# JOP-Lee/READ

Hardware: NVIDIA B200
Metric: frames/sec @1920x1080, 10M pts (higher is better)
Workload: dtype bf16

## Files before the change

read_b200/csrc/conv_tc.cu:

```cuda
#include "common.cuh"
#include "conv_common.cuh"
#include "ptx.cuh"
#include <cuda.h>
#include <mutex>
#include <new>

namespace rb {

#ifdef READ_DIAG
#define TC_DBG(a_, bit_) (((a_).debug & (bit_)) != 0)
#define TC_TRACE(role_, code_)                                                                                          \
    do {                                                                                                                \
        if (a.trace != nullptr && blockIdx.x == 0 && lane == 0 && trc_n < 2046u) {                                      \
            a.trace[(role_) * 2048 + 1 + trc_n] = ((unsigned long long)(code_) << 56) | ((unsigned long long)clock64() & 0x00FFFFFFFFFFFFFFull); \
            a.trace[(role_) * 2048] = ++trc_n;                                                                          \
        }                                                                                                               \
    } while (0)
#else
#define TC_DBG(a_, bit_) false
#define TC_TRACE(role_, code_) do { } while (0)
#endif

constexpr int TC_TW = 8, TC_TH = 16;
constexpr int TC_MAX_STAGES = 16;
constexpr uint32_t TC_SMEM_BUDGET = 218 * 1024;
constexpr uint32_t TC_RESIDENT_MAX = 144 * 1024;
constexpr int TC_TMEM_COLS = 512;
constexpr int TC_MAX_ACC = 8;
constexpr int BAR_AFULL = 0, BAR_AEMPTY = 16, BAR_BFULL = 32, BAR_BEMPTY = 48, BAR_TFULL = 64, BAR_TEMPTY = 72,
              BAR_BRES = 80, BAR_TMEMPTR = 82, BAR_RFULL = 84, BAR_PARAMS = 132;
constexpr int TC_STAGE_BYTES = 1024, TC_NBUF = 3;
constexpr uint32_t TC_STAGING_BYTES = 16u * TC_NBUF * TC_STAGE_BYTES;

struct TcMaps {
    CUtensorMap a[READ_MAX_SRC];
    CUtensorMap o, r;
};

struct TcArgs {
    int B, H, W, Cin, Cout, cout_pad;
    int ksize, pad;
    int cin_blk, kchunks;
    int n_tile, n_tiles;
    int tiles_x, tiles_y;
    int a_stages, b_stages, b_resident;
    int halo_w;
    uint32_t a_tx_bytes;
    uint32_t tile_bytes;
    int stride;
    int n_src;
    int src_kc_end[READ_MAX_SRC];
    int src_shift[READ_MAX_SRC];
    float inv_tx, inv_ty;
    int nacc;
    int dual;
    int debug;
    uint32_t a_bytes, b_bytes, b_region_off;
    int elu;
    const float *bias_f, *bias_m, *scale, *shift;
    const __nv_bfloat16 *residual;
    __nv_bfloat16 *out;
    float *out_nchw;
    __nv_bfloat16 *out2;
    const __nv_bfloat16 *out2_mul;
    const __nv_bfloat16 *addin;
    int addin_H, addin_W;
    int raw;
    int mt;
    int mt_log2, nacc_log2;
    int stiles_x;
    float inv_stx;
    int role_rot;
    int pdl;
    int commit_late;
    int merge_done;
    int bpair;
    int rev_total;
    int tma_out;
    uint32_t stage_bytes;
    int probe;
    unsigned long long *trace;
};

struct TileCoord {
    int nt, tx, ty, b;
};
__device__ __forceinline__ TileCoord decode_tile(long long t, const TcArgs &a)
{
    TileCoord c;
    if (a.rev_total) t = (long long)a.rev_total - 1 - t;
    int mt = (int)t;
    c.nt = 0;
    if (a.n_tiles == 2) { c.nt = mt & 1; mt >>= 1; }
    else if (a.n_tiles > 2) { c.nt = (int)(t % a.n_tiles); mt = (int)(t / a.n_tiles); }
    const int q = fdiv_small(mt, a.inv_stx);
    c.tx = (mt - q * a.stiles_x) * a.mt;
    c.b = fdiv_small(q, a.inv_ty);
    c.ty = q - c.b * a.tiles_y;
    return c;
}
__device__ __forceinline__ TileCoord decode_supertile(int s, const TcArgs &a)
{
    TileCoord c;
    c.nt = 0;
    if (a.rev_total) s = a.rev_total - 1 - s;
    const int q = fdiv_small(s, a.inv_stx);
    c.tx = (s - q * a.stiles_x) * a.mt;
    c.b = fdiv_small(q, a.inv_ty);
    c.ty = q - c.b * a.tiles_y;
    return c;
}
// ... 22 lines not shown
    extern __shared__ uint8_t smem_raw[];
    const uint32_t smem_base = (s_u32(smem_raw) + 1023u) & ~1023u;
    uint8_t *smem_al = smem_raw + (smem_base - s_u32(smem_raw));

    constexpr int ntaps = KS * KS;
    const uint32_t b_region = smem_base + a.b_region_off;
    const uint32_t b_region_bytes = RES ? (uint32_t)(ntaps * a.kchunks) * a.b_bytes : (uint32_t)a.b_stages * a.b_bytes;
    const uint32_t stage_region = smem_base + a.b_region_off + b_region_bytes;
    uint64_t *bars = reinterpret_cast<uint64_t *>(smem_al + a.b_region_off + b_region_bytes + a.stage_bytes);
    const uint32_t bar0 = s_u32(bars);
    const uint32_t afull0 = bar0 + 8 * BAR_AFULL, aempty0 = bar0 + 8 * BAR_AEMPTY;
    const uint32_t bfull0 = bar0 + 8 * BAR_BFULL, bempty0 = bar0 + 8 * BAR_BEMPTY;
    const uint32_t tfull0 = bar0 + 8 * BAR_TFULL, tempty0 = bar0 + 8 * BAR_TEMPTY, bres = bar0 + 8 * BAR_BRES;
    uint32_t *tmem_ptr_smem = reinterpret_cast<uint32_t *>(bars + BAR_TMEMPTR);
    float *s_par = reinterpret_cast<float *>(bars + BAR_PARAMS);

    const int lane = threadIdx.x & 31;
    const int warp = a.role_rot ? (int)(((threadIdx.x >> 5) + 4u) % (NTHR / 32)) : (int)(threadIdx.x >> 5);
    if (a.pdl) pdl_launch_dependents();
#ifdef READ_DIAG
    unsigned trc_n = 0;
#endif

    for (int i = threadIdx.x; i < a.cout_pad; i += NTHR) {
        const float hs = NTHR == 640 ? 0.5f : 1.f;
        reinterpret_cast<float4 *>(s_par)[i] = i < a.Cout ? make_float4(a.bias_f[i], hs * a.bias_m[i], hs * a.scale[i], a.shift[i])
                                                          : make_float4(0.f, 0.f, 0.f, 0.f);
    }
    if (warp == 0 && lane == 0) {
        for (int i = 0; i < a.n_src; ++i) tma_prefetch_desc(&tm.a[i]);
        tma_prefetch_desc(&tmB);
        if (a.tma_out) {
            tma_prefetch_desc(&tm.o);
            if (a.residual != nullptr) tma_prefetch_desc(&tm.r);
        }
    }
    if (warp == 1 && lane == 0) {
        for (int s = 0; s < TC_MAX_STAGES; ++s) {
            mbar_init(afull0 + 8 * s, 1);
            mbar_init(aempty0 + 8 * s, 1);
            mbar_init(bfull0 + 8 * s, 1);
            mbar_init(bempty0 + 8 * s, 1);
        }
        for (int i = 0; i < TC_MAX_ACC; ++i) {
            mbar_init(tfull0 + 8 * i, 1);
            mbar_init(tempty0 + 8 * i, NTHR == 640 ? (a.raw ? 16u : (uint32_t)(a.n_tile >> 3)) : ((a.n_tile >> 1) == 8 ? 4u : (NTHR - 128) / 32));
        }
        mbar_init(bres, 1);
        if (NTHR == 640)
            for (int i = 0; i < 16 * TC_NBUF; ++i) mbar_init(bar0 + 8 * (BAR_RFULL + i), 1);
        mbar_fence_init();
    }
    if (warp == 2) tmem_alloc(s_u32(tmem_ptr_smem), TC_TMEM_COLS);
    tcgen05_fence_before();
    __syncthreads();
    tcgen05_fence_after();
    const uint32_t tmem_base = *tmem_ptr_smem;

    const int m_tiles = a.stiles_x * a.tiles_y * a.B;
    const long long total_tiles = (long long)m_tiles * a.n_tiles;
    const int n_total = a.n_tile * a.n_tiles;

    if (warp == 0 || (warp == 2 && a.dual)) {
        const uint32_t pme = (warp == 2) ? 1u : 0u;
        if (RES && pme == 0u && elect_one()) {
            const int nb = KS * KS * a.kchunks;
            mbar_arrive_expect_tx(bres, (uint32_t)nb * a.b_bytes);
// ... 182 lines not shown
                        if (last_kc)
                            for (uint32_t mi = 0; mi < MT; ++mi) umma_commit(tfull0 + 8 * (acc + mi));
                    }
                    __syncwarp();
                }
                TC_TRACE(2 + me, 5);
                a_lo += st16;
                if (++as == ring_n) { as = 0; aph ^= 1u; a_lo = ring_lo0; }
            }
        }
    } else if (warp >= 4) {
        const int q = warp & 3;
        const int sub = (warp - 4) >> 2;
        const int r = q * 32 + lane;
        const int py = r / TC_TW, px = r % TC_TW;
        const int half = a.n_tile >> 1;
        const int nchunks = half >> 4;
        const float4 *par4 = reinterpret_cast<const float4 *>(s_par);
        unsigned tile_seq = 0;
        uint32_t acc_c = 0, acc_p = 0;
        if (a.pdl) pdl_wait();
        if (NTHR == 640 && (EPI != 0 || !a.raw)) {
            const bool elu = EPI == 1 ? true : (EPI == 2 ? false : a.elu != 0);
            const bool has_res = EPI == 2 ? true : (EPI == 1 ? false : a.residual != nullptr);
            const bool has_out2 = EPI != 0 ? false : a.out2 != nullptr;
            const int nch16 = half >> 4;
            const int lg = nch16 >> 1;
            const int chunk = sub & (nch16 - 1);
            const uint32_t item_step = 4u >> lg;
            const uint32_t n_units = (uint32_t)((total_tiles - blockIdx.x + gridDim.x - 1) / gridDim.x);
            const uint32_t n_mtiles = n_units << a.mt_log2;
            uint32_t acc = ((uint32_t)sub >> lg) % (uint32_t)a.nacc, acc_ph = (((uint32_t)sub >> lg) / (uint32_t)a.nacc) & 1u;
            const bool tma_out = a.tma_out != 0;
            const uint32_t sbuf0 = stage_region + (uint32_t)(warp - 4) * (TC_NBUF * TC_STAGE_BYTES);
            const uint32_t rfull0 = bar0 + 8 * (BAR_RFULL + (warp - 4) * TC_NBUF);
            const uint32_t lane_off = (uint32_t)lane * 32u, sw = (((uint32_t)lane >> 2) & 1u) * 16u;
            uint32_t kb = 0, kph = 0;
            if (tma_out && has_res && lane == 0 && ((uint32_t)sub >> lg) < n_mtiles) {
                const uint32_t it0 = (uint32_t)sub >> lg;
                const TileCoord t0 = decode_supertile((int)(blockIdx.x + (it0 >> a.mt_log2) * gridDim.x), a);
                mbar_arrive_expect_tx(rfull0, TC_STAGE_BYTES);
                tma_load_4d(&tm.r, rfull0, sbuf0, chunk * 16, (t0.tx + (int)(it0 & (uint32_t)(a.mt - 1))) * TC_TW, t0.ty * TC_TH + q * 4, t0.b);
            }
            for (uint32_t it = (uint32_t)sub >> lg; it < n_mtiles; it += item_step) {
                const uint32_t su = it >> a.mt_log2, mi = it & (uint32_t)(a.mt - 1);
                const TileCoord tc_ = decode_supertile((int)(blockIdx.x + su * gridDim.x), a);
                const int b = tc_.b;
                const int x = (tc_.tx + (int)mi) * TC_TW + px, y = tc_.ty * TC_TH + py;
                const bool inside = (x < a.W) && (y < a.H);
                const uint32_t trow = tmem_base + acc * (uint32_t)a.n_tile + ((uint32_t)(q * 32) << 16);
                const int co = chunk * 16;
                const int o = ((b * a.H + y) * a.W + x) * a.Cout + co;
                uint4 rs0 = make_uint4(0, 0, 0, 0), rs1 = rs0, ml0 = rs0, ml1 = rs0;
                uint4 af0 = rs0, af1 = rs0, am0 = rs0, am1 = rs0;
                const bool has_addin = EPI == 0 && a.addin != nullptr;
                if (has_addin && inside) {
                    const __nv_bfloat16 *ap = a.addin + ((b * a.addin_H + (y >> 1)) * a.addin_W + (x >> 1)) * a.n_tile + chunk * 16;
                    af0 = __ldg(reinterpret_cast<const uint4 *>(ap));
                    af1 = __ldg(reinterpret_cast<const uint4 *>(ap) + 1);
                    am0 = __ldg(reinterpret_cast<const uint4 *>(ap + half));
                    am1 = __ldg(reinterpret_cast<const uint4 *>(ap + half) + 1);
                }
                const uint32_t kn = kb + 1 == TC_NBUF ? 0u : kb + 1;
                if (tma_out) {
                    if (lane == 0) {
                        bulk_wait_group_read<1>();
                        const uint32_t itn = it + item_step;
                        if (has_res && itn < n_mtiles) {
                            const TileCoord tn = decode_supertile((int)(blockIdx.x + (itn >> a.mt_log2) * gridDim.x), a);
                            mbar_arrive_expect_tx(rfull0 + 8 * kn, TC_STAGE_BYTES);
                            tma_load_4d(&tm.r, rfull0 + 8 * kn, sbuf0 + kn * TC_STAGE_BYTES, co,
                                        (tn.tx + (int)(itn & (uint32_t)(a.mt - 1))) * TC_TW, tn.ty * TC_TH + q * 4, tn.b);
                        }
                    }
                } else if (inside) {
                    if (has_res) {
                        rs0 = __ldg(reinterpret_cast<const uint4 *>(a.residual + o));
                        rs1 = __ldg(reinterpret_cast<const uint4 *>(a.residual + o) + 1);
                    }
                    if (has_out2) {
                        ml0 = __ldg(reinterpret_cast<const uint4 *>(a.out2_mul + o));
                        ml1 = __ldg(reinterpret_cast<const uint4 *>(a.out2_mul + o) + 1);
                    }
                }
                TC_TRACE(warp, 9);
                mbar_wait(tfull0 + 8 * acc, acc_ph);
                TC_TRACE(warp, 6);
                tcgen05_fence_after();
                uint32_t f16[16], m16[16];
                tmem_ld16(trow + (uint32_t)(chunk * 16), f16);
                tmem_ld16(trow + (uint32_t)(half + chunk * 16), m16);
                tmem_ld_wait();
                TC_TRACE(warp, 7);
                tcgen05_fence_before();
                __syncwarp();
                if (lane == 0) mbar_arrive(tempty0 + 8 * acc);
                if (has_addin) {
                    const uint32_t fa[8] = {af0.x, af0.y, af0.z, af0.w, af1.x, af1.y, af1.z, af1.w};
                    const uint32_t ma[8] = {am0.x, am0.y, am0.z, am0.w, am1.x, am1.y, am1.z, am1.w};
#pragma unroll
                    for (int j = 0; j < 8; ++j) {
                        f16[2 * j] = __float_as_uint(__uint_as_float(f16[2 * j]) + __uint_as_float(fa[j] << 16));
                        f16[2 * j + 1] = __float_as_uint(__uint_as_float(f16[2 * j + 1]) + __uint_as_float(fa[j] & 0xFFFF0000u));
                        m16[2 * j] = __float_as_uint(__uint_as_float(m16[2 * j]) + __uint_as_float(ma[j] << 16));
                        m16[2 * j + 1] = __float_as_uint(__uint_as_float(m16[2 * j + 1]) + __uint_as_float(ma[j] & 0xFFFF0000u));
                    }
                }
                float yv[16];
                if (elu) {
#pragma unroll
                    for (int j = 0; j < 16; ++j) yv[j] = gate_folded<true>(__uint_as_float(f16[j]), __uint_as_float(m16[j]), par4[co + j]);
                } else {
#pragma unroll
                    for (int j = 0; j < 16; ++j) yv[j] = gate_folded<false>(__uint_as_float(f16[j]), __uint_as_float(m16[j]), par4[co + j]);
                }
                if (tma_out) {
                    const uint32_t sb = sbuf0 + kb * TC_STAGE_BYTES + lane_off;
                    if (has_res) {
                        mbar_wait(rfull0 + 8 * kb, kph);
                        asm volatile("ld.shared.v4.b32 {%0, %1, %2, %3}, [%4];" : "=r"(rs0.x), "=r"(rs0.y), "=r"(rs0.z), "=r"(rs0.w) : "r"(sb + sw));
                        asm volatile("ld.shared.v4.b32 {%0, %1, %2, %3}, [%4];" : "=r"(rs1.x), "=r"(rs1.y), "=r"(rs1.z), "=r"(rs1.w) : "r"(sb + (sw ^ 16u)));
                        const uint32_t rr[8] = {rs0.x, rs0.y, rs0.z, rs0.w, rs1.x, rs1.y, rs1.z, rs1.w};
#pragma unroll
                        for (int j = 0; j < 8; ++j) {
                            yv[2 * j] += __uint_as_float(rr[j] << 16);
                            yv[2 * j + 1] += __uint_as_float(rr[j] & 0xFFFF0000u);
                        }
                    }
                    uint32_t pk[8];
#pragma unroll
                    for (int j = 0; j < 8; ++j) pk[j] = cvt_bf16x2(yv[2 * j], yv[2 * j + 1]);
                    asm volatile("st.shared.v4.b32 [%0], {%1, %2, %3, %4};" ::"r"(sb + sw), "r"(pk[0]), "r"(pk[1]), "r"(pk[2]), "r"(pk[3]) : "memory");
                    asm volatile("st.shared.v4.b32 [%0], {%1, %2, %3, %4};" ::"r"(sb + (sw ^ 16u)), "r"(pk[4]), "r"(pk[5]), "r"(pk[6]), "r"(pk[7]) : "memory");
                    fence_proxy_async_smem();
                    __syncwarp();
                    if (lane == 0) {
                        if (!TC_DBG(a, 8)) tma_store_4d(&tm.o, sbuf0 + kb * TC_STAGE_BYTES, co, (tc_.tx + (int)mi) * TC_TW, tc_.ty * TC_TH + q * 4, b);
                        bulk_commit_group();
                    }
                    kb = kn;
                    if (kb == 0) kph ^= 1u;
                } else if (inside) {
                    if (has_res) {
                        const uint32_t rr[8] = {rs0.x, rs0.y, rs0.z, rs0.w, rs1.x, rs1.y, rs1.z, rs1.w};
#pragma unroll
                        for (int j = 0; j < 8; ++j) {
                            yv[2 * j] += __uint_as_float(rr[j] << 16);
                            yv[2 * j + 1] += __uint_as_float(rr[j] & 0xFFFF0000u);
                        }
                    }
                    uint32_t pk[8];
#pragma unroll
                    for (int j = 0; j < 8; ++j) pk[j] = cvt_bf16x2(yv[2 * j], yv[2 * j + 1]);
                    uint4 *op = reinterpret_cast<uint4 *>(a.out + o);
                    op[0] = make_uint4(pk[0], pk[1], pk[2], pk[3]);
                    op[1] = make_uint4(pk[4], pk[5], pk[6], pk[7]);
                    if (has_out2) {
                        const uint32_t mm[8] = {ml0.x, ml0.y, ml0.z, ml0.w, ml1.x, ml1.y, ml1.z, ml1.w};
                        uint32_t p2[8];
#pragma unroll
                        for (int j = 0; j < 8; ++j) {
                            const float2 ys = unpack_bf16x2(pk[j]);
                            const float2 mv = unpack_bf16x2(mm[j]);
                            p2[j] = cvt_bf16x2(ys.x * mv.x, ys.y * mv.y);
                        }
                        uint4 *o2 = reinterpret_cast<uint4 *>(a.out2 + o);
                        o2[0] = make_uint4(p2[0], p2[1], p2[2], p2[3]);
                        o2[1] = make_uint4(p2[4], p2[5], p2[6], p2[7]);
                    }
                }
                TC_TRACE(warp, 8);
// ... 168 lines not shown
        tmem_dealloc(tmem_base, TC_TMEM_COLS);
    }
}

__global__ void pack_tc_kernel(const float *__restrict__ wf, const float *__restrict__ wm, int Cout, int cout_pad, int Cin,
                               int k, int cin_blk, int n_tile, __nv_bfloat16 *__restrict__ out)
{
    const int kchunks = (Cin + cin_blk - 1) / cin_blk;
    const int n_total = 2 * cout_pad;
    const int half = n_tile / 2;
    const long long total = (long long)k * k * kchunks * n_total * cin_blk;
    for (long long i = blockIdx.x * (long long)blockDim.x + threadIdx.x; i < total;
         i += (long long)gridDim.x * blockDim.x) {
        const int kk = (int)(i % cin_blk);
        long long r = i / cin_blk;
        const int n = (int)(r % n_total);
        r /= n_total;
        const int kc = (int)(r % kchunks);
        const int tap = (int)(r / kchunks);
        const int nt = n / n_tile, rr = n % n_tile;
        const bool is_m = rr >= half;
        const int co = nt * half + (rr % half);
        const int c = kc * cin_blk + kk;
        const int ky = tap / k, kx = tap % k;
        const float *w = is_m ? wm : wf;
        out[i] = __float2bfloat16_rn((co < Cout && c < Cin) ? w[(((long long)co * Cin + c) * k + ky) * k + kx] : 0.f);
    }
}

struct TcGeom {
    int cin_blk, kchunks, n_tile, n_tiles, cout_pad;
};
int g_tc_commit_late = 0, g_tc_merge_done = 1, g_tc_bpair = 0, g_tc_probe = 0;
extern int g_tc_tma_store;
int g_tc_pair_wide = 1;
int g_tc_pair = 1;
int g_tc_mt = 1;
static int desc_chan_gran(const read_conv_desc &d)
{
    int gsrc = d.Cin;
    for (int i = 0; i < d.n_src && d.n_src > 1; ++i)
        if (d.src[i].C % 64 != 0) gsrc = 32;
    return gsrc;
}

static bool tc_geom(int Cin, int Cout, int stride, TcGeom *g, int chan_gran = 64)
{
    int cin_blk;
    if (Cin % 64 == 0 && stride == 1 && chan_gran % 64 == 0) cin_blk = 64;
    else if (Cin % 32 == 0) cin_blk = 32;
    else if ((Cin == 8 || Cin == 16) && stride == 1) cin_blk = 16;
    else return false;
    int cout_pad = Cout;
    if (Cout <= 8) cout_pad = 8;
    else if (Cout % 16 != 0) return false;
    const int n_total = 2 * cout_pad;
    const int n_tile = n_total <= 256 ? n_total : 256;
    if (n_total % n_tile != 0) return false;
    if (cout_pad > 8 && (n_tile / 2) % 16 != 0) return false;
    if (cin_blk == 16 && (n_total / n_tile != 1 || cout_pad <= 8 || !(cout_pad == 16 || cout_pad == 32 || cout_pad == 64))) return false;
    if (g) *g = TcGeom{cin_blk, (Cin + cin_blk - 1) / cin_blk, n_tile, n_total / n_tile, cout_pad};
    return true;
}

bool tc_supported(const read_conv_desc &d)
{
// ... 56 lines not shown
        cudaDriverEntryPointQueryResult qres;
        if (cudaGetDriverEntryPoint("cuTensorMapEncodeTiled", &p, cudaEnableDefault, &qres) == cudaSuccess &&
            qres == cudaDriverEntryPointSuccess)
            fn = reinterpret_cast<PFN_encodeTiled>(p);
    });
    return fn;
}

struct TcPlan {
    TcMaps tmA;
    CUtensorMap tmB;
    TcArgs args;
    size_t smem_bytes;
    Tc2Plan *pair;
    int reverse;
};

int tc_plan_create(const read_conv_desc &d, TcPlan **out)
{
    TcGeom g;
    if (!tc_supported(d) || !tc_geom(d.Cin, d.Cout, d.stride, &g, desc_chan_gran(d))) {
        set_error("tcgen05 conv: unsupported layer");
        return READ_ERR_UNSUPPORTED;
    }
    PFN_encodeTiled enc = get_encode_tiled();
    if (!enc) {
        set_error("tcgen05 conv: cuTensorMapEncodeTiled not available from the driver");
        return READ_ERR_CUDA;
    }
    RB_CHECK_ARG((reinterpret_cast<uintptr_t>(d.w_tc) & 127) == 0, "tcgen05 conv: packed weights must be 128B aligned");
    RB_CHECK_ARG((reinterpret_cast<uintptr_t>(d.out) & 15) == 0, "tcgen05 conv: output must be 16B aligned");
    RB_CHECK_ARG(d.residual == nullptr || (reinterpret_cast<uintptr_t>(d.residual) & 15) == 0, "tcgen05 conv: residual must be 16B aligned");
    RB_CHECK_ARG(d.addin == nullptr || (reinterpret_cast<uintptr_t>(d.addin) & 15) == 0, "tcgen05 conv: addin must be 16B aligned");
    TcPlan *p = new (std::nothrow) TcPlan{};
    RB_CHECK_ARG(p != nullptr, "tcgen05 conv: out of host memory");
    if (g_tc_pair && tc2_supported(d) && d.out_mode == READ_OUT_NHWC && (d.Cin == 64 || (d.Cin == 32 && d.residual == nullptr) || (d.Cin > 64 && g_tc_pair_wide) || g_tc_pair >= 2)) {
        const int rc2 = tc2_plan_create(d, &p->pair);
        if (rc2 != READ_OK) { delete p; return rc2; }
    }

    const bool s2 = d.stride == 2;
    const int halo_rows = s2 ? TC_TH + 1 : TC_TH + d.k - 1;
    const int tiles_x0 = (d.Wout + TC_TW - 1) / TC_TW;
    const int nacc0 = TC_TMEM_COLS / g.n_tile > TC_MAX_ACC ? TC_MAX_ACC : TC_TMEM_COLS / g.n_tile;
    int mt = 1;
    if (!s2 && g.n_tiles == 1) {
        const uint32_t total_b0 = (uint32_t)(d.k * d.k * g.kchunks) * (uint32_t)g.n_tile * g.cin_blk * 2u;
        const uint32_t ab1 = (((uint32_t)halo_rows * (uint32_t)(TC_TW + d.k - 1) * g.cin_blk * 2u) + 1023u) & ~1023u;
        const bool res1 = total_b0 <= TC_RESIDENT_MAX && TC_SMEM_BUDGET - total_b0 >= 2 * ab1;
        for (int cand = 4; cand >= 2; cand >>= 1) {
            if (g_tc_mt > 0 && cand != g_tc_mt) continue;
            if (cand * g.n_tile > 256 || nacc0 % cand != 0) continue;
            if (g_tc_mt <= 0 && tiles_x0 < 4 * cand) continue;
            const uint32_t ab = (((uint32_t)halo_rows * (uint32_t)(TC_TW * cand + d.k - 1) * g.cin_blk * 2u) + 1023u) & ~1023u;
            if (res1 ? ((TC_SMEM_BUDGET - total_b0) / ab < (uint32_t)(4 * g.kchunks))
                     : (3 * ab + 4u * (uint32_t)g.n_tile * g.cin_blk * 2u > TC_SMEM_BUDGET)) continue;
            mt = cand;
            break;
        }
        if (g_tc_mt == 1) mt = 1;
    }
    const int halo_w = s2 ? TC_TW + 1 : TC_TW * mt + d.k - 1;
    const CUtensorMapSwizzle sw = g.cin_blk == 64 ? CU_TENSOR_MAP_SWIZZLE_128B
                                  : (g.cin_blk == 32 ? CU_TENSOR_MAP_SWIZZLE_64B : CU_TENSOR_MAP_SWIZZLE_32B);
    for (int si = 0; si < d.n_src; ++si) {
        const read_src &sv = d.src[si];
// ... 31 lines not shown
    a.B = d.B; a.H = d.Hout; a.W = d.Wout; a.Cin = d.Cin; a.Cout = d.Cout; a.cout_pad = g.cout_pad;
    a.ksize = d.k; a.pad = d.pad;
    a.cin_blk = g.cin_blk; a.kchunks = g.kchunks; a.n_tile = g.n_tile; a.n_tiles = g.n_tiles;
    a.tiles_x = (d.Wout + TC_TW - 1) / TC_TW;
    a.tiles_y = (d.Hout + TC_TH - 1) / TC_TH;
    a.mt = mt;
    a.mt_log2 = mt == 4 ? 2 : (mt == 2 ? 1 : 0);
    a.stiles_x = (a.tiles_x + mt - 1) / mt;
    a.inv_stx = 1.0f / (float)a.stiles_x;
    a.halo_w = halo_w;
    a.stride = d.stride;
    a.n_src = d.n_src;
    {
        int kc = 0;
        for (int si = 0; si < READ_MAX_SRC; ++si) {
            int sh = 0;
            if (si < d.n_src) {
                kc += d.src[si].C / g.cin_blk;
                if (d.n_src > 1 && d.src[si].mode == READ_SRC_NEAREST_DOWN)
                    while ((1 << sh) < d.src[si].factor) ++sh;
            }
            a.src_kc_end[si] = kc;
            a.src_shift[si] = sh;
        }
    }
    a.a_tx_bytes = (uint32_t)halo_rows * halo_w * g.cin_blk * 2u;
    a.tile_bytes = (a.a_tx_bytes + 1023u) & ~1023u;
    a.a_bytes = s2 ? 4u * a.tile_bytes : a.tile_bytes;
    a.b_bytes = (uint32_t)g.n_tile * g.cin_blk * 2u;
    const uint32_t total_b = (uint32_t)(d.k * d.k * g.kchunks) * a.b_bytes;
    a.b_resident = (g.n_tiles == 1 && total_b <= TC_RESIDENT_MAX && TC_SMEM_BUDGET - total_b >= 2 * a.a_bytes) ? 1 : 0;
    uint32_t budget = TC_SMEM_BUDGET;
    a.tma_out = 0;
    a.stage_bytes = 0;
    {
        const int half_n = g.n_tile >> 1;
        const bool lean = (half_n == 16 || half_n == 32 || half_n == 64) && g.n_tiles == 1 && d.Cout == g.cout_pad &&
                          (long long)d.B * d.Hout * d.Wout * d.Cout < (1ll << 31);
        if (g_tc_tma_store && lean && d.out_mode == READ_OUT_NHWC && d.out2 == nullptr && budget > TC_STAGING_BYTES) {
            const uint32_t small = budget - TC_STAGING_BYTES;
            bool ok;
            if (a.b_resident) {
                const uint32_t full_st = (budget - total_b) / a.a_bytes, st = small > total_b ? (small - total_b) / a.a_bytes : 0;
                ok = st >= 2 && (st >= 6 || st >= full_st || st >= (uint32_t)TC_MAX_STAGES);
            } else {
                const uint32_t full_st = (budget - 3 * a.a_bytes) / a.b_bytes, st = small > 3 * a.a_bytes ? (small - 3 * a.a_bytes) / a.b_bytes : 0;
                ok = st >= 2 && (st >= 6 || st >= full_st || st >= (uint32_t)TC_MAX_STAGES);
            }
            if (ok) {
                a.tma_out = 1;
                a.stage_bytes = TC_STAGING_BYTES;
                budget = small;
            }
        }
    }
    uint32_t b_region_bytes;
    if (a.b_resident) {
        int st = (int)((budget - total_b) / a.a_bytes);
        a.a_stages = st > TC_MAX_STAGES ? TC_MAX_STAGES : st;
        a.b_stages = 0;
        b_region_bytes = total_b;
    } else {
        a.a_stages = 3;
        if (3 * a.a_bytes + 2 * a.b_bytes > budget) {
            set_error("tcgen05 conv: layer does not fit shared memory (A stage %u B, B tile %u B)", a.a_bytes, a.b_bytes);
            delete p;
            return READ_ERR_UNSUPPORTED;
        }
        int st = (int)((budget - 3 * a.a_bytes) / a.b_bytes);
        a.b_stages = st > TC_MAX_STAGES ? TC_MAX_STAGES : st;
        b_region_bytes = (uint32_t)a.b_stages * a.b_bytes;
    }
    if (a.tma_out) {
        cuuint64_t dims[4] = {(cuuint64_t)d.Cout, (cuuint64_t)d.Wout, (cuuint64_t)d.Hout, (cuuint64_t)d.B};
        cuuint64_t strides[3] = {(cuuint64_t)d.Cout * 2, (cuuint64_t)d.Wout * d.Cout * 2, (cuuint64_t)d.Hout * d.Wout * d.Cout * 2};
        cuuint32_t box[4] = {16, (cuuint32_t)TC_TW, 4, 1};
        cuuint32_t estr[4] = {1, 1, 1, 1};
        CUresult r = enc(&p->tmA.o, CU_TENSOR_MAP_DATA_TYPE_BFLOAT16, 4, d.out, dims, strides, box, estr, CU_TENSOR_MAP_INTERLEAVE_NONE,
                         CU_TENSOR_MAP_SWIZZLE_32B, CU_TENSOR_MAP_L2_PROMOTION_NONE, CU_TENSOR_MAP_FLOAT_OOB_FILL_NONE);
        if (r == CUDA_SUCCESS)
            r = enc(&p->tmA.r, CU_TENSOR_MAP_DATA_TYPE_BFLOAT16, 4, d.residual ? const_cast<void *>(d.residual) : d.out, dims, strides, box,
                    estr, CU_TENSOR_MAP_INTERLEAVE_NONE, CU_TENSOR_MAP_SWIZZLE_32B, CU_TENSOR_MAP_L2_PROMOTION_NONE,
                    CU_TENSOR_MAP_FLOAT_OOB_FILL_NONE);
        if (r != CUDA_SUCCESS) {
            set_error("tcgen05 conv: cuTensorMapEncodeTiled(output items) failed with %d", (int)r);
            delete p;
            return READ_ERR_CUDA;
        }
    }
    a.inv_tx = 1.0f / (float)a.tiles_x;
    a.inv_ty = 1.0f / (float)a.tiles_y;
    a.nacc = TC_TMEM_COLS / g.n_tile > TC_MAX_ACC ? TC_MAX_ACC : TC_TMEM_COLS / g.n_tile;
    a.nacc_log2 = 0;
    while ((1 << a.nacc_log2) < a.nacc) ++a.nacc_log2;
    a.dual = (a.b_resident && a.a_stages >= 4 * g.kchunks) ? 1 : 0;
    if (a.dual) a.a_stages &= ~1;
    a.commit_late = g_tc_commit_late ? 1 : 0;
    a.merge_done = 0;
    if (g_tc_merge_done && a.b_resident && g.kchunks == 1 && mt == 1 && a.a_stages >= 2) {
        a.merge_done = 1;
        const int depth = a.a_stages < a.nacc ? a.a_stages : a.nacc;
        a.dual = depth >= 4 ? 1 : 0;
        a.a_stages = a.nacc = a.dual ? (depth & ~1) : depth;
    }
    a.probe = (g_tc_probe && a.b_resident && g.kchunks == 1 && mt == 1) ? 1 : 0;
    a.bpair = 0;
    if (g_tc_bpair && !a.b_resident && a.b_stages >= 4) {
        a.bpair = 1;
        a.b_stages &= ~1;
        b_region_bytes = (uint32_t)a.b_stages * a.b_bytes;
    }
    a.b_region_off = (uint32_t)a.a_stages * a.a_bytes;
    a.elu = d.elu;
    a.bias_f = d.bias_f; a.bias_m = d.bias_m; a.scale = d.bn_scale; a.shift = d.bn_shift;
    a.residual = static_cast<const __nv_bfloat16 *>(d.residual);
    a.out = static_cast<__nv_bfloat16 *>(d.out);
// ... 163 lines not shown
```

read_b200/csrc/raster.cu:

```cuda
#include "common.cuh"
#include "ptx.cuh"
#include <string.h>

namespace rb {

constexpr int RP_THREADS = 256;
constexpr int RP_CHUNK = 1024;
constexpr int RP_STAGES = 3;
constexpr int RP_MAXB = 16;
constexpr int RP_STAGE_BYTES = RP_CHUNK * 12;

struct RasterArgs {
    const float *xyz;
    long long n;
    long long id_base;
    const float *M;
    int B, L;
    int w[READ_MAX_LEVELS], h[READ_MAX_LEVELS];
    float wf[READ_MAX_LEVELS], hf[READ_MAX_LEVELS];
    long long off[READ_MAX_LEVELS];
    unsigned direct_mask;
    unsigned long long *zbuf;
    int bulk_ok;
    int pipelined;
// ... 582 lines not shown
        unsigned long long m0 = k0 < k1 ? k0 : k1, m1 = k2 < k3 ? k2 : k3;
        coarse[i] = m0 < m1 ? m0 : m1;
    }
}

__global__ void zbuf_clear_kernel(unsigned long long *z, long long n)
{
    const long long stride = (long long)gridDim.x * blockDim.x;
    long long i = blockIdx.x * (long long)blockDim.x + threadIdx.x;
    if ((reinterpret_cast<uintptr_t>(z) & 15) == 0) {
        ulonglong2 *z2 = reinterpret_cast<ulonglong2 *>(z);
        const long long n2 = n >> 1;
        for (long long j = i; j < n2; j += stride) z2[j] = make_ulonglong2(ZBUF_EMPTY, ZBUF_EMPTY);
        if (i == 0 && (n & 1)) z[n - 1] = ZBUF_EMPTY;
    } else {
        for (long long j = i; j < n; j += stride) z[j] = ZBUF_EMPTY;
    }
}

__global__ void zbuf_resolve_kernel(const unsigned long long *__restrict__ z, long long n, float *__restrict__ index,
                                    float *__restrict__ depth)
{
    for (long long i = blockIdx.x * (long long)blockDim.x + threadIdx.x; i < n;
         i += (long long)gridDim.x * blockDim.x) {
        const unsigned long long k = z[i];
        const bool empty = (k == ZBUF_EMPTY);
        if (index) index[i] = empty ? 0.f : (float)(unsigned)(k & 0xFFFFFFFFull);
        if (depth) depth[i] = empty ? 0.f : __uint_as_float((unsigned)(k >> 32));
    }
}

extern int g_tc_debug, g_tcg_debug;
extern int g_gather_variant;
extern int g_tc_mt, g_tc_role_rot, g_tc_pdl, g_tc_commit_late, g_tc_merge_done, g_tc_bpair, g_tc_probe, g_tc_pair, g_tc_pair_wide, g_tc_tma_store, g_tc_wide_ntile;
int g_raster_pipelined = 1;
int g_raster_bulk = 1;
int g_raster_mode = 2;
int g_raster_occ = 0;
int g_raster_dedup = 0;
int g_raster_nbr = 0;
int g_raster_stream = 1;
int g_raster_stages = 2;
int g_raster_carveout = 45;
int g_raster_run = 0;

static unsigned direct_mask_of(const LevelGeom &g, int L)
{
    unsigned mask = 1u;
    for (int l = 1; l < L; ++l) {
        const bool nested = (g.w[l - 1] == 2 * g.w[l]) && (g.h[l - 1] == 2 * g.h[l]);
        if (!nested) mask |= (1u << l);
    }
    return mask;
}

static int launch_project(const float *xyz, long long n, long long id_base, const float *M, int B, int W, int H,
                          int L, unsigned long long *zbuf, cudaStream_t st)
{
    const LevelGeom g = level_geom(B, W, H, L);
    const size_t smem = (size_t)RP_STAGES * RP_STAGE_BYTES;
    RB_CUDA(cudaFuncSetAttribute(raster_project_kernel<true>, cudaFuncAttributeMaxDynamicSharedMemorySize, (int)smem));
    RB_CUDA(cudaFuncSetAttribute(raster_project_kernel<false>, cudaFuncAttributeMaxDynamicSharedMemorySize, (int)smem));
    for (int b0 = 0; b0 < B; b0 += RP_MAXB) {
        const int nb = (B - b0) < RP_MAXB ? (B - b0) : RP_MAXB;
        RasterArgs a{};
        a.xyz = xyz;
        a.n = n;
// ... 134 lines not shown
    if (h) *h = g.h[l];
}
unsigned read_raster_direct_mask(int W, int H, int L)
{
    if (L < 1 || L > READ_MAX_LEVELS) return 0;
    return direct_mask_of(level_geom(1, W, H, L), L);
}

int read_set_option(const char *name, int value)
{
    RB_CHECK_ARG(name != nullptr, "set_option: null name");
    if (!strcmp(name, "raster_pipelined")) { g_raster_pipelined = value; return READ_OK; }
    if (!strcmp(name, "raster_bulk_tma")) { g_raster_bulk = value; return READ_OK; }
    if (!strcmp(name, "raster_mode")) {
#ifndef READ_DIAG
        RB_CHECK_ARG(value >= 0 && value <= 3, "set_option: raster_mode %d is a wrong-output diagnostic (READ_DIAG builds only)", value);
#endif
        g_raster_mode = value;
        return READ_OK;
    }
#ifdef READ_DIAG
    if (!strcmp(name, "tc_debug")) { g_tc_debug = value; return READ_OK; }
    if (!strcmp(name, "tcg_debug")) { g_tcg_debug = value; return READ_OK; }
#endif
    if (!strcmp(name, "gather_variant")) { g_gather_variant = value; return READ_OK; }
    if (!strcmp(name, "tc_mt")) { g_tc_mt = value; return READ_OK; }
    if (!strcmp(name, "tc_role_rot")) { g_tc_role_rot = value; return READ_OK; }
    if (!strcmp(name, "tc_pdl")) { g_tc_pdl = value; return READ_OK; }
    if (!strcmp(name, "tc_commit_late")) { g_tc_commit_late = value; return READ_OK; }
    if (!strcmp(name, "tc_merge_done")) { g_tc_merge_done = value; return READ_OK; }
    if (!strcmp(name, "tc_bpair")) { g_tc_bpair = value; return READ_OK; }
    if (!strcmp(name, "tc_probe")) { g_tc_probe = value; return READ_OK; }
    if (!strcmp(name, "tc_tma_store")) { g_tc_tma_store = value; return READ_OK; }
    if (!strcmp(name, "tc_wide_ntile")) { g_tc_wide_ntile = value; return READ_OK; }
    if (!strcmp(name, "tc_pair_wide")) { g_tc_pair_wide = value; return READ_OK; }
    if (!strcmp(name, "tc_pair")) { g_tc_pair = value; return READ_OK; }
    if (!strcmp(name, "raster_occupancy")) { g_raster_occ = value; return READ_OK; }
    if (!strcmp(name, "raster_dedup")) { g_raster_dedup = value; return READ_OK; }
    if (!strcmp(name, "raster_run")) { g_raster_run = value; return READ_OK; }
    if (!strcmp(name, "raster_stream")) { g_raster_stream = value; return READ_OK; }
    if (!strcmp(name, "raster_stages")) { if (value != 2 && value != 3) { set_error("raster_stages: 2 or 3"); return READ_ERR_INVALID; } g_raster_stages = value; return READ_OK; }
    if (!strcmp(name, "raster_carveout")) { if (value < -1 || value > 100) { set_error("raster_carveout: -1..100"); return READ_ERR_INVALID; } g_raster_carveout = value; return READ_OK; }
    if (!strcmp(name, "raster_nbr_filter")) { g_raster_nbr = value; return READ_OK; }
    set_error("set_option: unknown option '%s'", name);
    return READ_ERR_INVALID;
}

int read_zbuf_clear(uint64_t *zbuf, int64_t entries, void *stream)
{
    RB_CHECK_ARG(entries >= 0, "read_zbuf_clear: negative size");
    if (entries == 0) return READ_OK;
    RB_CHECK_ARG(zbuf != nullptr, "read_zbuf_clear: null zbuf");
    long long blocks = (entries / 2 + 255) / 256;
    if (blocks < 1) blocks = 1;
    if (blocks > (long long)num_sms() * 16) blocks = (long long)num_sms() * 16;
    zbuf_clear_kernel<<<(unsigned)blocks, 256, 0, (cudaStream_t)stream>>>((unsigned long long *)zbuf, entries);
    RB_LAUNCH_CHECK();
    return READ_OK;
}

static int check_raster_args(const float *xyz, int64_t n, const float *M, int B, int W, int H, int L,
                             const uint64_t *zbuf)
{
    RB_CHECK_ARG(n >= 0, "raster: n must be >= 0");
    RB_CHECK_ARG(n == 0 || xyz != nullptr, "raster: in_points must be a CUDA tensor");
    RB_CHECK_ARG(M != nullptr && zbuf != nullptr, "raster: total_m / zbuf must be CUDA tensors");
// ... 125 lines not shown
```

Measured before the change: 161.9.

## Extend TMA-store epilogue to out2 and addin conv tails

Lets convolutions that have a second gated output (out2 = y * out2_mul) or an upsampled addin term use the TMA staged store path instead of per-thread global stores and loads. The multiplier or addin tile is prefetched with TMA into per-warp shared staging buffers, and both outputs are written with TMA stores. An extra staging buffer is reserved for the out2 case, so fewer A/B pipeline stages may fit. This adds barrier waits and shared-memory traffic in the epilogue warps.

Result: no change. 163.7, median of 6 (+1.1%).

```diff
diff --git a/read_b200/csrc/conv_tc.cu b/read_b200/csrc/conv_tc.cu
--- a/read_b200/csrc/conv_tc.cu
+++ b/read_b200/csrc/conv_tc.cu
@@ -31,10 +31,12 @@
               BAR_BRES = 80, BAR_TMEMPTR = 82, BAR_RFULL = 84, BAR_PARAMS = 132;
 constexpr int TC_STAGE_BYTES = 1024, TC_NBUF = 3;
 constexpr uint32_t TC_STAGING_BYTES = 16u * TC_NBUF * TC_STAGE_BYTES;
+constexpr uint32_t TC_STAGING_BYTES_OUT2 = 16u * (TC_NBUF + 1) * TC_STAGE_BYTES;
 
 struct TcMaps {
     CUtensorMap a[READ_MAX_SRC];
-    CUtensorMap o, r;
+    CUtensorMap o, o2;
+    CUtensorMap r;
 };
 
 struct TcArgs {
@@ -77,6 +79,7 @@
     int bpair;
     int rev_total;
     int tma_out;
+    int addin_tma;
     uint32_t stage_bytes;
     int probe;
     unsigned long long *trace;
@@ -165,7 +168,8 @@
         tma_prefetch_desc(&tmB);
         if (a.tma_out) {
             tma_prefetch_desc(&tm.o);
-            if (a.residual != nullptr) tma_prefetch_desc(&tm.r);
+            if (a.out2 != nullptr) tma_prefetch_desc(&tm.o2);
+            if (a.residual != nullptr || a.out2 != nullptr || a.addin_tma) tma_prefetch_desc(&tm.r);
         }
     }
     if (warp == 1 && lane == 0) {
@@ -414,16 +418,28 @@
             const uint32_t n_mtiles = n_units << a.mt_log2;
             uint32_t acc = ((uint32_t)sub >> lg) % (uint32_t)a.nacc, acc_ph = (((uint32_t)sub >> lg) / (uint32_t)a.nacc) & 1u;
             const bool tma_out = a.tma_out != 0;
-            const uint32_t sbuf0 = stage_region + (uint32_t)(warp - 4) * (TC_NBUF * TC_STAGE_BYTES);
+            const bool addin_tma = EPI == 0 && a.addin_tma != 0;
+            const bool side_tma = tma_out && (has_res || has_out2 || addin_tma);
+            const uint32_t sbuf0 = stage_region + (uint32_t)(warp - 4) * (a.stage_bytes >> 4);
+            const uint32_t ybuf = sbuf0 + TC_NBUF * TC_STAGE_BYTES;
             const uint32_t rfull0 = bar0 + 8 * (BAR_RFULL + (warp - 4) * TC_NBUF);
             const uint32_t lane_off = (uint32_t)lane * 32u, sw = (((uint32_t)lane >> 2) & 1u) * 16u;
+            const uint32_t add_off = (((uint32_t)lane >> 4) * 4u + (((uint32_t)lane & 7u) >> 1)) * 32u;
+            auto load_side = [&](uint32_t itx, uint32_t k) {
+                const TileCoord tn = decode_supertile((int)(blockIdx.x + (itx >> a.mt_log2) * gridDim.x), a);
+                const int x0 = (tn.tx + (int)(itx & (uint32_t)(a.mt - 1))) * TC_TW, y0 = tn.ty * TC_TH + q * 4;
+                const uint32_t bar = rfull0 + 8 * k, dst = sbuf0 + k * TC_STAGE_BYTES;
+                if (addin_tma) {
+                    mbar_arrive_expect_tx(bar, 2u * 256u);
+                    tma_load_4d(&tm.r, bar, dst, chunk * 16, x0 >> 1, y0 >> 1, tn.b);
+                    tma_load_4d(&tm.r, bar, dst + 256u, half + chunk * 16, x0 >> 1, y0 >> 1, tn.b);
+                } else {
+                    mbar_arrive_expect_tx(bar, TC_STAGE_BYTES);
+                    tma_load_4d(&tm.r, bar, dst, chunk * 16, x0, y0, tn.b);
+                }
+            };
             uint32_t kb = 0, kph = 0;
-            if (tma_out && has_res && lane == 0 && ((uint32_t)sub >> lg) < n_mtiles) {
-                const uint32_t it0 = (uint32_t)sub >> lg;
-                const TileCoord t0 = decode_supertile((int)(blockIdx.x + (it0 >> a.mt_log2) * gridDim.x), a);
-                mbar_arrive_expect_tx(rfull0, TC_STAGE_BYTES);
-                tma_load_4d(&tm.r, rfull0, sbuf0, chunk * 16, (t0.tx + (int)(it0 & (uint32_t)(a.mt - 1))) * TC_TW, t0.ty * TC_TH + q * 4, t0.b);
-            }
+            if (side_tma && lane == 0 && ((uint32_t)sub >> lg) < n_mtiles) load_side((uint32_t)sub >> lg, 0);
             for (uint32_t it = (uint32_t)sub >> lg; it < n_mtiles; it += item_step) {
                 const uint32_t su = it >> a.mt_log2, mi = it & (uint32_t)(a.mt - 1);
                 const TileCoord tc_ = decode_supertile((int)(blockIdx.x + su * gridDim.x), a);
@@ -436,7 +452,7 @@
                 uint4 rs0 = make_uint4(0, 0, 0, 0), rs1 = rs0, ml0 = rs0, ml1 = rs0;
                 uint4 af0 = rs0, af1 = rs0, am0 = rs0, am1 = rs0;
                 const bool has_addin = EPI == 0 && a.addin != nullptr;
-                if (has_addin && inside) {
+                if (has_addin && !addin_tma && inside) {
                     const __nv_bfloat16 *ap = a.addin + ((b * a.addin_H + (y >> 1)) * a.addin_W + (x >> 1)) * a.n_tile + chunk * 16;
                     af0 = __ldg(reinterpret_cast<const uint4 *>(ap));
                     af1 = __ldg(reinterpret_cast<const uint4 *>(ap) + 1);
@@ -448,12 +464,7 @@
                     if (lane == 0) {
                         bulk_wait_group_read<1>();
                         const uint32_t itn = it + item_step;
-                        if (has_res && itn < n_mtiles) {
-                            const TileCoord tn = decode_supertile((int)(blockIdx.x + (itn >> a.mt_log2) * gridDim.x), a);
-                            mbar_arrive_expect_tx(rfull0 + 8 * kn, TC_STAGE_BYTES);
-                            tma_load_4d(&tm.r, rfull0 + 8 * kn, sbuf0 + kn * TC_STAGE_BYTES, co,
-                                        (tn.tx + (int)(itn & (uint32_t)(a.mt - 1))) * TC_TW, tn.ty * TC_TH + q * 4, tn.b);
-                        }
+                        if (side_tma && itn < n_mtiles) load_side(itn, kn);
                     }
                 } else if (inside) {
                     if (has_res) {
@@ -477,6 +488,15 @@
                 tcgen05_fence_before();
                 __syncwarp();
                 if (lane == 0) mbar_arrive(tempty0 + 8 * acc);
+                if (addin_tma) {
+                    mbar_wait(rfull0 + 8 * kb, kph);
+                    const uint32_t ab = sbuf0 + kb * TC_STAGE_BYTES + add_off;
+                    asm volatile("ld.shared.v4.b32 {%0, %1, %2, %3}, [%4];" : "=r"(af0.x), "=r"(af0.y), "=r"(af0.z), "=r"(af0.w) : "r"(ab));
+                    asm volatile("ld.shared.v4.b32 {%0, %1, %2, %3}, [%4];" : "=r"(af1.x), "=r"(af1.y), "=r"(af1.z), "=r"(af1.w) : "r"(ab + 16u));
+                    asm volatile("ld.shared.v4.b32 {%0, %1, %2, %3}, [%4];" : "=r"(am0.x), "=r"(am0.y), "=r"(am0.z), "=r"(am0.w) : "r"(ab + 256u));
+                    asm volatile("ld.shared.v4.b32 {%0, %1, %2, %3}, [%4];" : "=r"(am1.x), "=r"(am1.y), "=r"(am1.z), "=r"(am1.w) : "r"(ab + 272u));
+                    __syncwarp();
+                }
                 if (has_addin) {
                     const uint32_t fa[8] = {af0.x, af0.y, af0.z, af0.w, af1.x, af1.y, af1.z, af1.w};
                     const uint32_t ma[8] = {am0.x, am0.y, am0.z, am0.w, am1.x, am1.y, am1.z, am1.w};
@@ -509,16 +529,39 @@
                             yv[2 * j + 1] += __uint_as_float(rr[j] & 0xFFFF0000u);
                         }
                     }
+                    if (has_out2) {
+                        mbar_wait(rfull0 + 8 * kb, kph);
+                        asm volatile("ld.shared.v4.b32 {%0, %1, %2, %3}, [%4];" : "=r"(ml0.x), "=r"(ml0.y), "=r"(ml0.z), "=r"(ml0.w) : "r"(sb + sw));
+                        asm volatile("ld.shared.v4.b32 {%0, %1, %2, %3}, [%4];" : "=r"(ml1.x), "=r"(ml1.y), "=r"(ml1.z), "=r"(ml1.w) : "r"(sb + (sw ^ 16u)));
+                    }
                     uint32_t pk[8];
 #pragma unroll
                     for (int j = 0; j < 8; ++j) pk[j] = cvt_bf16x2(yv[2 * j], yv[2 * j + 1]);
-                    asm volatile("st.shared.v4.b32 [%0], {%1, %2, %3, %4};" ::"r"(sb + sw), "r"(pk[0]), "r"(pk[1]), "r"(pk[2]), "r"(pk[3]) : "memory");
-                    asm volatile("st.shared.v4.b32 [%0], {%1, %2, %3, %4};" ::"r"(sb + (sw ^ 16u)), "r"(pk[4]), "r"(pk[5]), "r"(pk[6]), "r"(pk[7]) : "memory");
+                    const uint32_t yb = has_out2 ? ybuf + lane_off : sb;
+                    asm volatile("st.shared.v4.b32 [%0], {%1, %2, %3, %4};" ::"r"(yb + sw), "r"(pk[0]), "r"(pk[1]), "r"(pk[2]), "r"(pk[3]) : "memory");
+                    asm volatile("st.shared.v4.b32 [%0], {%1, %2, %3, %4};" ::"r"(yb + (sw ^ 16u)), "r"(pk[4]), "r"(pk[5]), "r"(pk[6]), "r"(pk[7]) : "memory");
+                    if (has_out2) {
+                        const uint32_t mm[8] = {ml0.x, ml0.y, ml0.z, ml0.w, ml1.x, ml1.y, ml1.z, ml1.w};
+                        uint32_t p2[8];
+#pragma unroll
+                        for (int j = 0; j < 8; ++j) {
+                            const float2 ys = unpack_bf16x2(pk[j]);
+                            const float2 mv = unpack_bf16x2(mm[j]);
+                            p2[j] = cvt_bf16x2(ys.x * mv.x, ys.y * mv.y);
+                        }
+                        asm volatile("st.shared.v4.b32 [%0], {%1, %2, %3, %4};" ::"r"(sb + sw), "r"(p2[0]), "r"(p2[1]), "r"(p2[2]), "r"(p2[3]) : "memory");
+                        asm volatile("st.shared.v4.b32 [%0], {%1, %2, %3, %4};" ::"r"(sb + (sw ^ 16u)), "r"(p2[4]), "r"(p2[5]), "r"(p2[6]), "r"(p2[7]) : "memory");
+                    }
                     fence_proxy_async_smem();
                     __syncwarp();
                     if (lane == 0) {
-                        if (!TC_DBG(a, 8)) tma_store_4d(&tm.o, sbuf0 + kb * TC_STAGE_BYTES, co, (tc_.tx + (int)mi) * TC_TW, tc_.ty * TC_TH + q * 4, b);
+                        const int ox = (tc_.tx + (int)mi) * TC_TW, oy = tc_.ty * TC_TH + q * 4;
+                        if (!TC_DBG(a, 8)) tma_store_4d(&tm.o, has_out2 ? ybuf : sbuf0 + kb * TC_STAGE_BYTES, co, ox, oy, b);
                         bulk_commit_group();
+                        if (has_out2) {
+                            if (!TC_DBG(a, 8)) tma_store_4d(&tm.o2, sbuf0 + kb * TC_STAGE_BYTES, co, ox, oy, b);
+                            bulk_commit_group();
+                        }
                     }
                     kb = kn;
                     if (kb == 0) kph ^= 1u;
@@ -753,6 +796,7 @@
     int cin_blk, kchunks, n_tile, n_tiles, cout_pad;
 };
 int g_tc_commit_late = 0, g_tc_merge_done = 1, g_tc_bpair = 0, g_tc_probe = 0;
+int g_tc_tma_tail = 1;
 extern int g_tc_tma_store;
 int g_tc_pair_wide = 1;
 int g_tc_pair = 1;
@@ -875,6 +919,8 @@
     RB_CHECK_ARG((reinterpret_cast<uintptr_t>(d.out) & 15) == 0, "tcgen05 conv: output must be 16B aligned");
     RB_CHECK_ARG(d.residual == nullptr || (reinterpret_cast<uintptr_t>(d.residual) & 15) == 0, "tcgen05 conv: residual must be 16B aligned");
     RB_CHECK_ARG(d.addin == nullptr || (reinterpret_cast<uintptr_t>(d.addin) & 15) == 0, "tcgen05 conv: addin must be 16B aligned");
+    RB_CHECK_ARG(d.out2 == nullptr || ((reinterpret_cast<uintptr_t>(d.out2) | reinterpret_cast<uintptr_t>(d.out2_mul)) & 15) == 0,
+                 "tcgen05 conv: out2 / out2_mul must be 16B aligned");
     TcPlan *p = new (std::nothrow) TcPlan{};
     RB_CHECK_ARG(p != nullptr, "tcgen05 conv: out of host memory");
     if (g_tc_pair && tc2_supported(d) && d.out_mode == READ_OUT_NHWC && (d.Cin == 64 || (d.Cin == 32 && d.residual == nullptr) || (d.Cin > 64 && g_tc_pair_wide) || g_tc_pair >= 2)) {
@@ -972,24 +1018,30 @@
     a.b_resident = (g.n_tiles == 1 && total_b <= TC_RESIDENT_MAX && TC_SMEM_BUDGET - total_b >= 2 * a.a_bytes) ? 1 : 0;
     uint32_t budget = TC_SMEM_BUDGET;
     a.tma_out = 0;
+    a.addin_tma = 0;
     a.stage_bytes = 0;
     {
         const int half_n = g.n_tile >> 1;
         const bool lean = (half_n == 16 || half_n == 32 || half_n == 64) && g.n_tiles == 1 && d.Cout == g.cout_pad &&
                           (long long)d.B * d.Hout * d.Wout * d.Cout < (1ll << 31);
-        if (g_tc_tma_store && lean && d.out_mode == READ_OUT_NHWC && d.out2 == nullptr && budget > TC_STAGING_BYTES) {
-            const uint32_t small = budget - TC_STAGING_BYTES;
+        const int n_side = (d.residual != nullptr) + (d.out2 != nullptr) + (d.addin != nullptr);
+        const bool tail_ok = g_tc_tma_tail || d.out2 == nullptr;
+        const uint32_t staging = d.out2 ? TC_STAGING_BYTES_OUT2 : TC_STAGING_BYTES;
+        if (g_tc_tma_store && tail_ok && lean && d.out_mode == READ_OUT_NHWC && n_side <= 1 && budget > staging) {
+            const uint32_t small = budget - staging;
+            const bool fam = d.out2 != nullptr;
             bool ok;
             if (a.b_resident) {
                 const uint32_t full_st = (budget - total_b) / a.a_bytes, st = small > total_b ? (small - total_b) / a.a_bytes : 0;
-                ok = st >= 2 && (st >= 6 || st >= full_st || st >= (uint32_t)TC_MAX_STAGES);
+                ok = st >= 2 && (st >= 6 || st >= full_st || st >= (uint32_t)TC_MAX_STAGES || fam);
             } else {
                 const uint32_t full_st = (budget - 3 * a.a_bytes) / a.b_bytes, st = small > 3 * a.a_bytes ? (small - 3 * a.a_bytes) / a.b_bytes : 0;
-                ok = st >= 2 && (st >= 6 || st >= full_st || st >= (uint32_t)TC_MAX_STAGES);
+                ok = st >= 2 && (st >= 6 || st >= full_st || st >= (uint32_t)TC_MAX_STAGES || fam);
             }
             if (ok) {
                 a.tma_out = 1;
-                a.stage_bytes = TC_STAGING_BYTES;
+                a.addin_tma = (d.addin != nullptr && g_tc_tma_tail) ? 1 : 0;
+                a.stage_bytes = staging;
                 budget = small;
             }
         }
@@ -1016,12 +1068,23 @@
         cuuint64_t strides[3] = {(cuuint64_t)d.Cout * 2, (cuuint64_t)d.Wout * d.Cout * 2, (cuuint64_t)d.Hout * d.Wout * d.Cout * 2};
         cuuint32_t box[4] = {16, (cuuint32_t)TC_TW, 4, 1};
         cuuint32_t estr[4] = {1, 1, 1, 1};
-        CUresult r = enc(&p->tmA.o, CU_TENSOR_MAP_DATA_TYPE_BFLOAT16, 4, d.out, dims, strides, box, estr, CU_TENSOR_MAP_INTERLEAVE_NONE,
-                         CU_TENSOR_MAP_SWIZZLE_32B, CU_TENSOR_MAP_L2_PROMOTION_NONE, CU_TENSOR_MAP_FLOAT_OOB_FILL_NONE);
-        if (r == CUDA_SUCCESS)
-            r = enc(&p->tmA.r, CU_TENSOR_MAP_DATA_TYPE_BFLOAT16, 4, d.residual ? const_cast<void *>(d.residual) : d.out, dims, strides, box,
-                    estr, CU_TENSOR_MAP_INTERLEAVE_NONE, CU_TENSOR_MAP_SWIZZLE_32B, CU_TENSOR_MAP_L2_PROMOTION_NONE,
+        auto item_map = [&](CUtensorMap *m, const void *ptr) {
+            return enc(m, CU_TENSOR_MAP_DATA_TYPE_BFLOAT16, 4, const_cast<void *>(ptr), dims, strides, box, estr,
+                       CU_TENSOR_MAP_INTERLEAVE_NONE, CU_TENSOR_MAP_SWIZZLE_32B, CU_TENSOR_MAP_L2_PROMOTION_NONE,
+                       CU_TENSOR_MAP_FLOAT_OOB_FILL_NONE);
+        };
+        CUresult r = item_map(&p->tmA.o, d.out);
+        if (r == CUDA_SUCCESS) r = item_map(&p->tmA.o2, d.out2 ? d.out2 : d.out);
+        if (r == CUDA_SUCCESS && a.addin_tma) {
+            cuuint64_t adims[4] = {(cuuint64_t)g.n_tile, (cuuint64_t)d.addin_W, (cuuint64_t)d.addin_H, (cuuint64_t)d.B};
+            cuuint64_t astr[3] = {(cuuint64_t)g.n_tile * 2, (cuuint64_t)d.addin_W * g.n_tile * 2, (cuuint64_t)d.addin_H * d.addin_W * g.n_tile * 2};
+            cuuint32_t abox[4] = {16, (cuuint32_t)TC_TW / 2, 2, 1};
+            r = enc(&p->tmA.r, CU_TENSOR_MAP_DATA_TYPE_BFLOAT16, 4, const_cast<void *>(d.addin), adims, astr, abox, estr,
+                    CU_TENSOR_MAP_INTERLEAVE_NONE, CU_TENSOR_MAP_SWIZZLE_NONE, CU_TENSOR_MAP_L2_PROMOTION_NONE,
                     CU_TENSOR_MAP_FLOAT_OOB_FILL_NONE);
+        } else if (r == CUDA_SUCCESS) {
+            r = item_map(&p->tmA.r, d.residual ? d.residual : (d.out2 ? d.out2_mul : d.out));
+        }
         if (r != CUDA_SUCCESS) {
             set_error("tcgen05 conv: cuTensorMapEncodeTiled(output items) failed with %d", (int)r);
             delete p;
diff --git a/read_b200/csrc/raster.cu b/read_b200/csrc/raster.cu
--- a/read_b200/csrc/raster.cu
+++ b/read_b200/csrc/raster.cu
@@ -638,7 +638,7 @@
 
 extern int g_tc_debug, g_tcg_debug;
 extern int g_gather_variant;
-extern int g_tc_mt, g_tc_role_rot, g_tc_pdl, g_tc_commit_late, g_tc_merge_done, g_tc_bpair, g_tc_probe, g_tc_pair, g_tc_pair_wide, g_tc_tma_store, g_tc_wide_ntile;
+extern int g_tc_mt, g_tc_role_rot, g_tc_pdl, g_tc_commit_late, g_tc_merge_done, g_tc_bpair, g_tc_probe, g_tc_pair, g_tc_pair_wide, g_tc_tma_store, g_tc_tma_tail, g_tc_wide_ntile;
 int g_raster_pipelined = 1;
 int g_raster_bulk = 1;
 int g_raster_mode = 2;
@@ -839,6 +839,7 @@
     if (!strcmp(name, "tc_bpair")) { g_tc_bpair = value; return READ_OK; }
     if (!strcmp(name, "tc_probe")) { g_tc_probe = value; return READ_OK; }
     if (!strcmp(name, "tc_tma_store")) { g_tc_tma_store = value; return READ_OK; }
+    if (!strcmp(name, "tc_tma_tail")) { g_tc_tma_tail = value; return READ_OK; }
     if (!strcmp(name, "tc_wide_ntile")) { g_tc_wide_ntile = value; return READ_OK; }
     if (!strcmp(name, "tc_pair_wide")) { g_tc_pair_wide = value; return READ_OK; }
     if (!strcmp(name, "tc_pair")) { g_tc_pair = value; return READ_OK; }
```
